# Julia-Tempering/Pigeons.jl

Hardware: AMD Instinct MI355X
Metric: replica-steps/sec (explore+swap), toy_mvn d=1024, n_chains=1024; round-trip rate (higher is better)
Workload: dtype f64

## Files before the change

include/pte.h:

```cpp
#ifndef PTE_H
#define PTE_H

#include <stdint.h>
#include "pte_rng_policy.h"

#ifdef __cplusplus
extern "C" {
#endif

#define PTE_ABI_VERSION 2

enum {
    PTE_TARGET_MVN_SCALED_PRECISION = 0,
    PTE_TARGET_TEST_SWAPPER         = 1,
    PTE_TARGET_FUNNEL               = 2,
    PTE_TARGET_ISING                = 3,
    PTE_TARGET_GAUSSIAN_MIXTURE     = 4,
    PTE_TARGET_BAYESIAN_GLM         = 5,
    PTE_TARGET_MIXTURE_MODEL        = 6,
    PTE_TARGET_VARIABLE_SELECTION = 7,
    PTE_TARGET_CHANGE_POINT = 8,
    PTE_TARGET_HIERARCHICAL_NORMAL = 9,
    PTE_TARGET_LATENT_AR1 = 10,
    PTE_TARGET_DENSE_NORMAL = 11,
// ... 23 lines not shown
    PTE_EXPLORER_CHECKERBOARD_METROPOLIS = 7
};
enum {
    PTE_RECORD_ROUND_TRIP    = 1u << 0,
    PTE_RECORD_INDEX_PROCESS = 1u << 1,
    PTE_RECORD_ONLINE        = 1u << 2,
    PTE_RECORD_TRACES        = 1u << 3,
    PTE_RECORD_TRACES_EXTENDED = 1u << 5,
    PTE_RECORD_ENERGY_AC1    = 1u << 4,
    PTE_RECORD_REFERENCE_REDUCTION = 1u << 6
};

enum {
    PTE_KERNEL_DEFAULT          = 0,
    PTE_KERNEL_SLICE_SEQUENTIAL = 1,
    PTE_KERNEL_ISING_BITS       = 101,
    PTE_KERNEL_ISING_BYTES      = 102,
    PTE_KERNEL_TWO_LAUNCHES     = 0x1000,
    PTE_KERNEL_SCAN_LOOP_ONE_CHAIN = 0x2000,
    PTE_KERNEL_FLAG_BITS        = 0x3000,
    PTE_KERNEL_TEST_DEAD_CHAIN     = 0x4000,
    PTE_KERNEL_TEST_LATE_WORKGROUP = 0x8000,
    PTE_KERNEL_TEST_LANGEVIN_ONE_WAVE = 0x10000,
    PTE_KERNEL_TEST_BITS        = 0x1C000
};

typedef struct pte_config {
    uint32_t struct_size;
    uint32_t abi_version;
    int32_t  device;
    int32_t  target;
    int32_t  explorer;
    uint32_t record_flags;
    int64_t  n_chains;
    int64_t  dim;
    uint64_t seed;
    int64_t  max_scans_per_round;
    double   target_params[4];
    double   slice_w;
    int32_t  slice_p;
    int32_t  slice_n_passes;
    int32_t  slice_max_iter;
    int32_t  am_base_n_refresh;
    double   am_exponent_n_refresh;
    double   am_step_size;
    double   am_p0, am_p1;
    int32_t  am_preconditioner;
// ... 70 lines not shown
int64_t pte_shard_message_bytes(const pte_engine *h);
int pte_shard_set_buffers(pte_engine *h, void *send_lo, void *recv_lo, void *send_hi, void *recv_hi);
int pte_shard_scan_begin(pte_engine *h, int64_t scan, int32_t *active_out);
int pte_shard_scan_finish(pte_engine *h, int64_t scan);
int pte_shard_sync(pte_engine *h, int64_t *boundary_swaps_out);
#define PTE_COMM_ID_BYTES 128
int pte_comm_allow_library_override(int32_t allow);
int pte_comm_library(char *path_out, int64_t capacity, int32_t *version_out);
int pte_comm_unique_id(uint8_t *id_out );
int pte_comm_init(pte_engine *h, const uint8_t *id );
int pte_comm_destroy(pte_engine *h);
int pte_comm_info(pte_engine *h, int32_t *kind, int32_t *n_ranks_seen, int64_t *boundary_swaps);
int pte_comm_barrier(pte_engine *h);
int pte_comm_allreduce(pte_engine *h, double *inout, int64_t n, int32_t op);
int pte_comm_allgather(pte_engine *h, const void *send, int64_t bytes, void *recv);
int pte_group_run_scans(pte_engine *const *engines, int32_t n_engines, int64_t first_scan, int64_t n_scans);

const char *pte_kernel_name(const pte_engine *h);

const char *pte_scan_loop_name(const pte_engine *h);
int pte_scan_loop_info(const pte_engine *h, int64_t *resident_limit, int64_t *timed_launches, int64_t *timed_scans);
int pte_scan_loop_stats(const pte_engine *h, int64_t *fused_calls, int64_t *gate_aborts, int32_t *poisoned);

int pte_get_index_process_shard(const pte_engine *h, int64_t *replica, int64_t *chain, int64_t *n_scans);
int pte_get_replica_ids(const pte_engine *h, int64_t *out );

int pte_timing_reset(pte_engine *h, int enable);
int pte_timing_get(const pte_engine *h, int kernel, double *total_ms, int64_t *launches);
int pte_timing_get_samples(const pte_engine *h, int kernel, double *out_ms, int64_t capacity, int64_t *n_out);

int pte_set_rng_policy(int32_t device, uint32_t policy);
int pte_get_rng_policy(int32_t device, uint32_t *policy);

int pte_test_rng_fill(int32_t device, uint64_t *seed_gamma , int32_t kind, int64_t n, double *out);
int pte_test_quotient(int32_t device, const double *a, const double *b, int64_t n, double *out, int32_t *took_division);
int pte_test_sqr_norm(int32_t device, const double *x, int64_t rows, int64_t d, double *out);

#ifdef __cplusplus
}
#endif
#endif
```

pigeons.jl_amd/csrc/pte.hip:

```cpp
#include <hip/hip_runtime.h>
#include <hip/hip_ext.h>

#include <cmath>
#include <cstdarg>
#include <cstdio>
#include <cstdlib>
#include <cstring>
#include <string>
#include <vector>

#include "../../include/pte.h"
#include "pte_kernels.hpp"
#include "pte_slice2.hpp"
#include "pte_slice5.hpp"
#include "pte_slice7.hpp"
#include "pte_slice8.hpp"
#ifdef PTE_SPLIT_LANGEVIN
#include "pte_automala_params.hpp"
#include "pte_aaps_params.hpp"
#include "pte_mixture_params.hpp"
#include "pte_glm_params.hpp"
#include "pte_hier_params.hpp"
#include "pte_ar1_params.hpp"
#include "pte_dense_params.hpp"
// ... 488 lines not shown
    hipLaunchKernelGGL(k_log_energy, dim3((unsigned)((N + 255) / 256)), dim3(256), 0, h->stream, h->dev, 1);
    HIP_OK(h, hipGetLastError());
    return 0;
}

int launch_explorer_kind(pte_engine *h, int64_t scan, int kind) {
    const int64_t N = h->K;
    switch (kind) {
    case PTE_EXPLORER_NONE: return 0;
    case PTE_EXPLORER_TOY:
        time_begin(h, 0, true);
        DISPATCH_NLU(h->nlu, k_explore_toy, dim3((unsigned)((N + NRM_WPB - 1) / NRM_WPB)), dim3(64 * NRM_WPB), h->stream, h->dev);
        time_end(h);
        break;
    case PTE_EXPLORER_SLICE:
        if (on_interpolated_path(h->cfg.target)) {
            const AmParams ap = slice_path_params(h);
            time_begin(h, 0, true);
            if (launch_path_kernel(h, blocks_per_lane(h->d), true, false, N, ap)) return 1;
            time_end(h);
            break;
        }
        {
        SliceParams sp{h->cfg.slice_w, h->cfg.slice_p, h->cfg.slice_n_passes, h->cfg.slice_max_iter};
        time_begin(h, 0, true);
        if (h->slice_impl == 1) {
            DISPATCH_NLU(h->nlu, k_explore_slice, dim3((unsigned)N), dim3(64), h->stream, h->dev, sp);
        } else if (h->slice_impl == 8) {
            const bool fast_ok = sp.p > PTE_S8_BD && sp.p <= 20 && sp.max_iter >= PTE_S8_BS;
            if (N <= PTE_S8_TWIN_FROM && fast_ok) { DISPATCH_NLU_M(h->nlu, k_explore_slice8, PTE_S8_BS, dim3((unsigned)N), dim3(64), h->stream, h->dev, sp); }
            else if (N <= PTE_S8_TWIN_FROM) { DISPATCH_NLU_M(h->nlu, k_explore_slice8_generic, PTE_S8_BS, dim3((unsigned)N), dim3(64), h->stream, h->dev, sp); }
            else { DISPATCH_NLU_M(h->nlu, k_explore_slice8_lds10k, PTE_S8_BS, dim3((unsigned)N), dim3(64), h->stream, h->dev, sp); }
        }
#ifdef PTE_TEST_KERNELS
        else if (h->slice_impl == 7) {
            S7Tune tn{2, 8, 2};
            DISPATCH_NLU(h->nlu, k_explore_slice7, dim3((unsigned)N), dim3(64), h->stream, h->dev, sp, tn);
        } else if (h->slice_impl == 5) {
            DISPATCH_NLU_M(h->nlu, k_explore_slice5, 4, dim3((unsigned)N), dim3(64), h->stream, h->dev, sp);
        } else if (h->slice_impl == 2) {
            DISPATCH_NLU_M(h->nlu, k_explore_slice2, 4, dim3((unsigned)N), dim3(64), h->stream, h->dev, sp);
        }
#endif
        else return fail(h, "SliceSampler kernel %d is not in this build", h->slice_impl);
        time_end(h);
        break;
    }
// ... 170 lines not shown
}

int run_scans_two_launches(pte_engine *h, int64_t first_scan, int64_t n_scans) {
    for (int64_t s = first_scan; s < first_scan + n_scans; ++s) {
        if (launch_explore(h, s)) return 1;
        if (launch_swap(h, s)) return 1;
    }
    int rc = check_device_error(h);
    time_collect(h);
    return rc;
}

int run_scans_fused(pte_engine *h, int64_t first_scan, int64_t n_scans) {
    const int64_t N = h->K;
    const int kind = fused_kind(h);
    const unsigned long long wgs = (unsigned long long)((kind == 2 && h->fused_wg > 1) ? (N + h->fused_wg - 1) / h->fused_wg : N);
    h->gate_seq += 1;
    ScanLoop sl{first_scan, n_scans, h->scans_in_round, h->hs_epoch, h->hs_flag, h->hs_pub, h->hs_gate, h->gate_seq, h->gate_arrived + wgs, h->test_fault};
    h->gate_arrived += wgs;
    h->dev.compose_phase = 0; h->dev.trace_idx = h->scans_in_round;
    time_begin(h, 4, true);
    const bool timed = h->ev_open;
    if (kind == 1) {
        SliceParams sp{h->cfg.slice_w, h->cfg.slice_p, h->cfg.slice_n_passes, h->cfg.slice_max_iter};
        if (fused_slice_variant(h) == 0) { DISPATCH_NLU_M(h->nlu, k_scans_slice8, PTE_S8_BS, dim3((unsigned)N), dim3(64), h->stream, h->dev, sp, sl); }
        else { DISPATCH_NLU_M(h->nlu, k_scans_slice8_generic, PTE_S8_BS, dim3((unsigned)N), dim3(64), h->stream, h->dev, sp, sl); }
    } else {
        const AmParams ap = langevin_params(h, h->cfg.explorer, 1);
        const int E = blocks_per_lane(h->d);
        LangevinLaunch L{E, h->cfg.target == PTE_TARGET_FUNNEL ? TGT_FUNNEL : TGT_MVN, false, h->d == 64 * (int64_t)E, launch_site(h, (unsigned)wgs)};
        L.scans = &sl; L.scan_wg = h->fused_wg;
        if (E == 16) HIP_OK(h, hipMemsetAsync(h->dev.pace, 0, sizeof(unsigned int), h->stream));
        if (langevin_launch(L, h->dev, ap)) { time_end(h); return fail(h, "this build holds no fused Langevin-family kernel"); }
    }
    time_end(h);
    HIP_OK(h, hipGetLastError());
    unsigned long long gate[2] = {0, 0};
    HIP_OK(h, hipMemcpyAsync(gate, h->hs_gate, sizeof gate, hipMemcpyDeviceToHost, h->stream));
    int rc = check_device_error(h);
    if (gate[1] == ((h->gate_seq << 1) | 1ull)) {
        if (timed && !h->events.empty() && h->events.back().kernel == 4) {
            h->ev_pool.push_back(h->events.back().a); h->ev_pool.push_back(h->events.back().b); h->events.pop_back();
        }
        h->gate_aborts += 1;
        h->fused_backoff = h->fused_backoff ? std::min<int64_t>(256, 2 * h->fused_backoff) : 1;
        h->fused_skip = h->fused_backoff;
        if (rc) return rc;
// ... 294 lines not shown
        auto composable = [&](int k) { return k == PTE_EXPLORER_SLICE || grad_based(k); };
        if (!composable(cfg->explorer) || !composable(cfg->explorer2))
            return fail(nullptr, "pte_create: Compose is available for SliceSampler / AutoMALA / MALA (got %d, %d)", cfg->explorer, cfg->explorer2);
    }
    if (!swapper && !ising && (cfg->dim < 1 || cfg->dim > 4096))
        return fail(nullptr, "pte_create: dim must be in 1..4096 (got %lld)", (long long)cfg->dim);
    if (swapper && cfg->explorer != PTE_EXPLORER_NONE)
        return fail(nullptr, "pte_create: TestSwapper has no explorer");
    if (!swapper && !ising && cfg->explorer != PTE_EXPLORER_TOY && cfg->explorer != PTE_EXPLORER_SLICE && !grad_based(cfg->explorer) && !aaps)
        return fail(nullptr, "pte_create: explorer %d is not implemented on the device", cfg->explorer);
    if ((cfg->record_flags & PTE_RECORD_TRACES_EXTENDED) && !(cfg->record_flags & PTE_RECORD_TRACES))
        return fail(nullptr, "pte_create: PTE_RECORD_TRACES_EXTENDED needs PTE_RECORD_TRACES");
    if (cfg->record_flags & PTE_RECORD_REFERENCE_REDUCTION) {
        if (!(cfg->record_flags & PTE_RECORD_INDEX_PROCESS))
            return fail(nullptr, "pte_create: PTE_RECORD_REFERENCE_REDUCTION needs PTE_RECORD_INDEX_PROCESS (the replay asks which replica held the lower chain of a pair)");
        if ((double)cfg->max_scans_per_round * (double)(cfg->n_chains + cfg->n_chains_variational) * 16.0 > 64e9)
            return fail(nullptr, "pte_create: the swap log (max_scans_per_round x chains x 2 doubles) would exceed 64 GB");
    }
#ifndef PTE_TEST_KERNELS
    if (cfg->debug_kernel & PTE_KERNEL_TEST_BITS)
        return fail(nullptr, "pte_create: debug_kernel 0x%x carries a fault-injection flag (PTE_KERNEL_TEST_*); those exist in the test build libpte_test.so only", cfg->debug_kernel);
#endif
    {
        const int dk = cfg->debug_kernel & ~(PTE_KERNEL_FLAG_BITS | PTE_KERNEL_TEST_BITS);
        const bool slice = cfg->explorer == PTE_EXPLORER_SLICE || cfg->explorer2 == PTE_EXPLORER_SLICE;
        bool ok = dk == 0 || (slice && dk == PTE_KERNEL_SLICE_SEQUENTIAL) || (ising && dk == PTE_KERNEL_ISING_BYTES);
#ifdef PTE_TEST_KERNELS
        ok = ok || (slice && (dk == 2 || dk == 5 || dk == 7 || dk == 8)) || (ising && !spin_glass && !checkerboard && dk == PTE_KERNEL_ISING_BITS);
#endif
        if (!ok) return fail(nullptr, "pte_create: debug_kernel %d is not available for this explorer in this build of libpte "
                                      "(0 = default, %d = sequential SliceSampler kernel; the other generations live in the test build libpte_test.so)",
                             dk, PTE_KERNEL_SLICE_SEQUENTIAL);
    }
    if ((cfg->record_flags & PTE_RECORD_TRACES) &&
        (double)cfg->max_scans_per_round * (double)((cfg->record_flags & PTE_RECORD_TRACES_EXTENDED) ? cfg->n_chains / cfg->world_size : 1) * (double)(cfg->dim + 1) * 8.0 > 64e9)
        return fail(nullptr, "pte_create: the traces buffer (max_scans_per_round x chains x (dim+1) doubles) would exceed 64 GB");
    return 0;
}

int poisoned_error(pte_engine *h, const char *what) {
    return fail(h, "%s: this engine is poisoned -- an earlier pte_run_scans failed inside the one-launch scan loop, its replicas stopped at different scans; "
                   "restore it with pte_set_state(state, chain, rng) or destroy it", what);
}
#define PTE_ALIVE(h, what) do { if ((h)->poisoned) return poisoned_error(h, what); } while (0)

int setter_entry(pte_engine *h, const char *setter, int32_t target, const char *wrong_target) {
    if (!h) return 1;
    PTE_ALIVE(h, setter);
// ... 53 lines not shown
const char *pte_last_error(const pte_engine *h) { return h ? h->err.c_str() : g_create_error.c_str(); }

int pte_create(const pte_config *cfg, pte_engine **out) {
    if (!cfg || !out) return fail(nullptr, "pte_create: null argument");
    *out = nullptr;
    if (validate_config(cfg)) return 1;
    int ndev = 0;
    if (hipGetDeviceCount(&ndev) != hipSuccess || ndev <= 0)
        return fail(nullptr, "pte_create: no HIP device available (this library has no CPU fallback)");
    if (cfg->device < 0 || cfg->device >= ndev) return fail(nullptr, "pte_create: bad device ordinal %d", cfg->device);

    pte_engine *h = new pte_engine();
    h->cfg = *cfg;
    const int64_t N = h->N = cfg->n_chains + cfg->n_chains_variational;
    const int64_t d = h->d = cfg->target == PTE_TARGET_TEST_SWAPPER ? 0 : cfg->dim;
    h->world = cfg->world_size; h->rank = cfg->rank;
    const int64_t K = h->K = N / cfg->world_size;
    h->c0 = K * cfg->rank;
    auto bail = [&](int) { g_create_error = h->err; pte_destroy(h); return 1; };
    if (hipSetDevice(cfg->device) != hipSuccess) { h->err = "hipSetDevice failed"; return bail(1); }
    if (hipStreamCreate(&h->stream) != hipSuccess) { h->err = "hipStreamCreate failed"; return bail(1); }
    const int64_t B = (d + 63) / 64;
    h->nlu = next_pow2_log(B > 0 ? B : 1);
    const int dk_kernel = cfg->debug_kernel & ~(PTE_KERNEL_FLAG_BITS | PTE_KERNEL_TEST_BITS);
    h->fused_allowed = (cfg->debug_kernel & PTE_KERNEL_TWO_LAUNCHES) == 0;
    h->fused_wg_allowed = (cfg->debug_kernel & PTE_KERNEL_SCAN_LOOP_ONE_CHAIN) == 0;
    h->test_fault = (cfg->debug_kernel & PTE_KERNEL_TEST_DEAD_CHAIN) ? 1 : ((cfg->debug_kernel & PTE_KERNEL_TEST_LATE_WORKGROUP) ? 2 : 0);
    if (cfg->explorer == PTE_EXPLORER_SLICE || cfg->explorer2 == PTE_EXPLORER_SLICE) h->slice_impl = dk_kernel == 0 ? 8 : dk_kernel;
    if (cfg->explorer == PTE_EXPLORER_ISING_METROPOLIS || cfg->explorer == PTE_EXPLORER_CHECKERBOARD_METROPOLIS) h->ising_impl = dk_kernel == PTE_KERNEL_ISING_BITS ? 1 : (dk_kernel == PTE_KERNEL_ISING_BYTES ? 2 : 0);
    if (alloc_engine(h)) return bail(1);
    default_schedule(h);
    if (upload_ladder(h)) return bail(1);
    if (reset_recorders(h)) return bail(1);
    if (init_replicas(h)) return bail(1);
    if ((on_interpolated_path(cfg->target) || on_lattice(cfg->target)) && init_zero_state(h)) return bail(1);
    *out = h;
    return 0;
}

int pte_destroy(pte_engine *h) {
    if (!h) return 0;
    hipSetDevice(h->cfg.device);
    if (h->stream) hipStreamSynchronize(h->stream);
    time_collect(h);
    pte_comm_destroy(h);
    if (h->ev_pack) hipEventDestroy(h->ev_pack);
    if (h->ev_copied) hipEventDestroy(h->ev_copied);
// ... 806 lines not shown
}

const char *pte_scan_loop_name(const pte_engine *hc) {
    pte_engine *h = const_cast<pte_engine *>(hc);
    if (!h) return "";
    hipSetDevice(h->cfg.device);
    if (!fused_scans_eligible(h, 1)) return "";
    if (fused_kind(h) == 2) return h->d > 512 ? "k_scans_langevin_mw" : h->fused_wg > 1 ? "k_scans_automala_wg" : "k_scans_automala";
    return fused_slice_variant(h) == 0 ? "k_scans_slice8" : "k_scans_slice8_generic";
}
int pte_scan_loop_info(const pte_engine *hc, int64_t *resident_limit, int64_t *timed_launches, int64_t *timed_scans) {
    pte_engine *h = const_cast<pte_engine *>(hc);
    if (!h) return 1;
    hipSetDevice(h->cfg.device);
    (void)fused_scans_eligible(h, 1);
    hipStreamSynchronize(h->stream);
    time_collect(h);
    if (resident_limit) *resident_limit = h->fused_limit < 0 ? 0 : h->fused_limit;
    if (timed_launches) *timed_launches = h->t_n[4];
    if (timed_scans) *timed_scans = h->t_scans4;
    return 0;
}

int pte_scan_loop_stats(const pte_engine *h, int64_t *fused_calls, int64_t *gate_aborts, int32_t *poisoned) {
    if (!h) return 1;
    if (fused_calls) *fused_calls = h->fused_calls;
    if (gate_aborts) *gate_aborts = h->gate_aborts;
    if (poisoned) *poisoned = h->poisoned ? 1 : 0;
    return 0;
}

int pte_set_target_mixture(pte_engine *h, int64_t n_components, const double *weights, const double *means, const double *std_devs) {
    if (setter_entry(h, "pte_set_target_mixture", PTE_TARGET_GAUSSIAN_MIXTURE, "pte_set_target_mixture: this engine's target is %d, not PTE_TARGET_GAUSSIAN_MIXTURE")) return 1;
    if (n_components < 1 || n_components > 8)
        return fail(h, "pte_set_target_mixture: the device holds 1..8 components (got %lld)", (long long)n_components);
    if (!weights || !means || !std_devs) return fail(h, "pte_set_target_mixture: null argument");
    const int64_t K = n_components, d = h->d, ld = h->dev.ld;
    for (int64_t k = 0; k < K; ++k) {
        if (!(weights[k] > 0) || !std::isfinite(weights[k]))
            return fail(h, "pte_set_target_mixture: weight %lld must be positive and finite (got %g)", (long long)k, weights[k]);
        for (int64_t i = 0; i < d; ++i) {
            const double sd = std_devs[k * d + i], mu = means[k * d + i];
            if (!(sd > 0) || !std::isfinite(sd))
                return fail(h, "pte_set_target_mixture: std_devs[%lld][%lld] must be positive and finite (got %g)", (long long)k, (long long)i, sd);
            if (!std::isfinite(mu))
                return fail(h, "pte_set_target_mixture: means[%lld][%lld] must be finite (got %g)", (long long)k, (long long)i, mu);
// ... 578 lines not shown
```

pigeons.jl_amd/csrc/pte_kernels.hpp:

```cpp
#pragma once
#include "pte_device.hpp"
#include "pte_normals.hpp"

namespace pte {

enum { ERR_NONE = 0, ERR_NAN_RATIO = 1, ERR_SLICE_SUPPORT = 2, ERR_SLICE_INVALID_LP = 3, ERR_SLICE_MAX_ITER = 4 };

struct EngineDev {
    int64_t N, d, ld;
    int64_t sw;
    int64_t K, c0;
    int64_t *replica_id;
    double *stat;
    double *nbr_stat;
    int32_t *bflag;
    int32_t *slot_of_chain_alt;
    int32_t *ip_replica;
    double *x;
    uint64_t *rng;
    int32_t *chain_of_slot;
    int32_t *slot_of_chain;
    double *suff;
    const double *nhp;
    const double *sd;
// ... 7 lines not shown
    double *swap_sum;  int64_t *swap_n;
    double *lsr_up;    double *lsr_dn;   int64_t *lsr_n;
    double *swap_log;
    int16_t *am_log; int am_log_cap;
    int64_t *rt_state; int64_t *rt_restarts; int64_t *rt_trips;
    double *expl_acc_sum; int64_t *expl_acc_n;
    double *expl_steps_sum; int64_t *expl_steps_n;
    double *on_mean; double *on_m2; int64_t *on_n;
    double *eac_log;
    double *eac; int64_t *eac_n;
    double *traces; int64_t trace_idx;
    int64_t ref2, tgt_a, tgt_b, rt_tgt_a, rt_tgt_b;
    const int32_t *v_use; const double *v_mean, *v_std, *v_c0, *v_i2, *v_gf; double *suff3;
    int compose_phase; double *lp_stash;
    int32_t *index_process;
    int32_t *error;
    double *mw_gk;
    unsigned int *pace;
    uint32_t record_flags;
    int32_t target;
    double test_swapper_pr;
};

struct SliceParams { double w; int p; int n_passes; int max_iter; };

__device__ __forceinline__ bool is_ref_chain(const EngineDev &e, int64_t c) { return (c == 0 && e.N > 1) || c == e.ref2; }
__device__ __forceinline__ bool is_tgt_chain(const EngineDev &e, int64_t c) { return c == e.tgt_a || c == e.tgt_b; }

__device__ __forceinline__ void set_error(const EngineDev &e, int code, int chain, int coord) {
    if (atomicCAS(&e.error[0], 0, code) == 0) { e.error[1] = chain; e.error[2] = coord; }
}

template <int NLU>
__global__ __launch_bounds__(64 * NRM_WPB) NRM_ATTR void k_init(EngineDev e, uint64_t master_seed, double init_sd) {
    __shared__ NormalsLds L;
    const int lane = lane_id();
    normals_lds_init(L, lane);
    const int64_t il = (int64_t)blockIdx.x * NRM_WPB + (NRM_WPB > 1 ? __builtin_amdgcn_readfirstlane((int)(threadIdx.x >> 6)) : 0);
    if (il >= e.K) return;
    const int64_t i = e.c0 + il;
    const uint64_t G = 0x9e3779b97f4a7c15ULL;
    SeqRng r;
    r.seed = mix64(master_seed + (uint64_t)(2 * i + 1) * G);
    r.gamma = mix_gamma(master_seed + (uint64_t)(2 * i + 2) * G);
    if (e.d > 0) {
        const double S = upper_tree_root<NLU>(normals_row(L, r, e.x + il * e.ld, e.d, init_sd, lane));
        if (lane == 0) e.suff[il] = S;
// ... 806 lines not shown
```

pigeons.jl_amd/csrc/pte_slice7.hpp:

```cpp
#pragma once
#include "pte_slice5.hpp"

namespace pte {

namespace s7 {
#ifndef PTE_S7_G
#define PTE_S7_G 5
#endif
constexpr int G = PTE_S7_G;
#ifndef PTE_S7_WIN
#define PTE_S7_WIN 512
#endif
constexpr int WIN = PTE_S7_WIN;
#ifndef PTE_S7_MARGIN
#define PTE_S7_MARGIN 80
#endif
constexpr int REFILL_AT = WIN - PTE_S7_MARGIN;
constexpr int CAP_ITERS = 24;
#ifndef PTE_S7_TABLES
#define PTE_S7_TABLES {0, 3, 6, 10, 14}, {1, 14, 16, 17, 16}, {0, 1, 15, 31, 48}
#endif
struct S7Tables { int lo[G], wd[G], base[G]; };
constexpr S7Tables S7T = {PTE_S7_TABLES};
struct S7Row { int v[G]; };
constexpr S7Row s7_row(const int (&a)[G]) { S7Row r{}; for (int i = 0; i < G; ++i) r.v[i] = a[i]; return r; }
__device__ constexpr S7Row LO_ = s7_row(S7T.lo), WD_ = s7_row(S7T.wd), BASE_ = s7_row(S7T.base);
#define LO LO_.v
#define WD WD_.v
#define BASE BASE_.v
__device__ __forceinline__ int s7_level(int lane) { int g = 0; for (int k = 1; k < G; ++k) g += (lane >= BASE[k]) ? 1 : 0; return g; }
__device__ __forceinline__ int s7_pick(const int (&a)[G], int g, int dflt) { int r = dflt; for (int k = 0; k < G; ++k) r = (g == k) ? a[k] : r; return r; }
constexpr int VALID = 1 << 30;
}

struct S7Tune { int bud_d, bud_s, bud_a; };
namespace s7 {
}

template <int NLU>
__global__ __launch_bounds__(64) void k_explore_slice7(EngineDev e, SliceParams sp, S7Tune tn) {
    using namespace s7;
    __shared__ double s_we[256];
    __shared__ unsigned long long s_ke[256];
    __shared__ double s_u[WIN];
    __shared__ double s_e[WIN];
    const int lane = lane_id();
    for (int i = lane; i < 256; i += 64) { s_we[i] = ZIG_WE[i]; s_ke[i] = ZIG_KE[i]; }
    __syncthreads();
    const int64_t cl = blockIdx.x;
    if (cl >= e.K) return;
    const int64_t c = e.c0 + cl;
    const int slot = e.slot_of_chain[cl];
// ... 294 lines not shown
```

pigeons.jl_amd/csrc/pte_slice8.hpp:

```cpp
#pragma once
#include "pte_slice7.hpp"

namespace pte {

#ifndef PTE_S8_BD
#define PTE_S8_BD 3
#endif
#ifndef PTE_S8_BS
#define PTE_S8_BS 9
#endif
constexpr int S8_BD = PTE_S8_BD;

#ifndef PTE_S8_WAVES
#define PTE_S8_WAVES 4
#endif
template <int NLU, int S8_BS, int WINDOW, int DBL_MODE>
__device__ __forceinline__ void slice8_body(EngineDev e, SliceParams sp, const int64_t cl) {
    using namespace s7;
    constexpr int WIN = WINDOW, REFILL_AT = WINDOW - PTE_S7_MARGIN;
    constexpr bool FAST = (DBL_MODE == 2);
    static_assert(CAP_ITERS >= S8_BS, "lane 0 must be able to run past the speculative budget");
#ifndef PTE_S8_BLK
#define PTE_S8_BLK 256
#endif
// ... 26 lines not shown
    __syncthreads();
    if (cl >= e.K) return;
    const int64_t c = e.c0 + cl;
    const int slot = e.slot_of_chain[cl];
    if (is_ref_chain(e, c)) {
        iid_refresh_recorded<NLU>(e, cl, c, slot, e.sd[c], lane);
        return;
    }
    const double lp_before = lp_before_explore(e, c, slot);
    const int64_t d = e.d;
    double *xrow = e.x + (int64_t)slot * e.ld;
    const int B = (int)((d + 63) >> 6);
    const double nhp = e.nhp[c];
    const double inv_nhp = 1.0 / nhp;
    const double inv_abs_nhp = -inv_nhp * (1.0 + 1e-6);
    const double w = sp.w;
    const double w11 = 1.1 * sp.w;
    const int cap_iters = min(sp.max_iter, CAP_ITERS);
    const int kcap = min(sp.p, 20);
    const bool shr_more = S8_BS < cap_iters;
    constexpr bool HAND_SHRINK = (S8_BS == PTE_S8_BS && S8_BS >= 6 && S8_BS <= 10);
    constexpr bool N_IS_KN = (DBL_MODE == 2) && HAND_SHRINK;

    const int hg = s7_level(lane);
    const int hrel = s7_pick(LO, hg, 0) + lane - s7_pick(BASE, hg, 0);

    const int succ_lo = s7_pick(LO, hg + 1, 0), succ_wd = s7_pick(WD, hg + 1, 0), succ_base = s7_pick(BASE, hg + 1, 0);
    const int succ_off = hrel - succ_lo;
    const int word_c = 0x10000 - succ_off;
    const int word_c9 = (1 << 20) - succ_off * 512;
    const uint64_t seed_in = e.rng[2 * slot];

    double BS = 0.0;
    for (int b = 0; b < B; ++b) {
        int64_t i = 64 * (int64_t)b + lane;
        double v = (i < d) ? xrow[i] : 0.0;
        double s = wave_sum_dpp(v * v);
        if (lane == b) BS = s;
    }
    double S = upper_tree_root<NLU>(BS);
    if (nhp * S == -INFINITY) { if (lane == 0) set_error(e, ERR_SLICE_SUPPORT, (int)c, -1); return; }

    uint64_t wseed = e.rng[2 * slot];
    const uint64_t gamma = e.rng[2 * slot + 1];
    int p = 0;
    uint64_t gamma_inv = gamma;
    for (int k = 0; k < 5; ++k) gamma_inv *= 2ull - gamma * gamma_inv;
    double wsum = 0.0;
    typedef unsigned mask2_t __attribute__((ext_vector_type(2)));
    typedef unsigned slow_mask_t __attribute__((ext_vector_type(WIN / 32)));
    typedef double draws8_t __attribute__((ext_vector_type(8)));
// ... 538 lines not shown
                                 : [sB] "=&s"(sB_), [tm] "=&s"(tmask), [acc] "=&s"(acc),
                                   [s0] "=&s"(s0_), [s1] "=&s"(s1_), [s2] "=&s"(s2_), [s3] "=&s"(s3_), [s4] "=&s"(s4_)
                                 : [w] "v"(w_), [pk] "v"(pk_)
                                 : "scc");
                    if (__builtin_amdgcn_inverse_ballot_w64(tmask)) s_x[(l + hg) & (BLK - 1)] = xf;
                    __builtin_amdgcn_wave_barrier();
                    p += (int)((acc >> 9) & 0x1FFu);
                    gdone = (int)((acc >> 20) & 7u);
                    l += gdone;
                } else {
                bool valid = __builtin_amdgcn_inverse_ballot_w64(pre_ok) && fin && (W > thr2);
                if constexpr (!FAST) valid = valid && !(E != E) && n <= cap_iters;
#ifdef PTE_PROFILE_SECTIONS
                asm volatile("" :: "v"(xf), "v"(n), "v"(dmin));
#endif
#ifdef PTE_PROFILE_SECTIONS
                {
                    const bool mg = dmin > 2e-12 * Bq;
                    const int rc = !active ? 7 : (E != E) ? 1 : !dbl_ok ? 2 : !fin ? 3 : !valid ? 4 : !mg ? 5 : 0;
                    const int cnt_ = N_IS_KN ? n - succ_off : cnt_base + kd + n;
                    int o_ = 0, g_ = 0, why = 0;
                    for (g_ = 0; g_ < G; ++g_) {
                        if (l + g_ >= nl) { why = 7; break; }
                        const int k_ = o_ - LO[g_];
                        if ((unsigned)k_ >= (unsigned)WD[g_]) { why = 6; break; }
                        const int ln_ = BASE[g_] + k_;
                        const int r_ = __builtin_amdgcn_readlane(rc, ln_);
                        if (r_) { why = r_; break; }
                        o_ += __builtin_amdgcn_readlane(cnt_, ln_);
                    }
                    PROF_ADD(8 + why, 1);
                }
#endif
                valid = valid && (dmin > mthr);
                const int kn = N_IS_KN ? n : kn0 + n;
                const bool inw = (unsigned)kn < (unsigned)succ_wd;
                const uint64_t vmask = ballot64(valid);
                int word_v = kn + word_c + (inw ? (int)((unsigned)(kn + succ_base) << 24) : 0);
                asm("" : "+v"(word_v));
                const int word = valid ? word_v : 0;
                const int packed = (lane != 0) ? word : 0;
#ifdef PTE_PROFILE_SECTIONS
                asm volatile("" :: "v"(packed));
#endif
                {
                    int pk = __builtin_amdgcn_readlane(word, 0);
                    unsigned acc = 0u;
                    uint64_t tmask = 1ull;
#pragma unroll
// ... 190 lines not shown
```

pigeons.jl_amd/pigeons_amd/_lib.py:

```python
import ctypes as C
import os

_HERE = os.path.dirname(os.path.abspath(__file__))
PKG_ROOT = os.path.dirname(_HERE)
LIB_PATH = os.path.join(PKG_ROOT, "lib", "libpte.so")


def use_library(path):
    global LIB_PATH
    LIB_PATH = path

TARGET_MVN_SCALED_PRECISION, TARGET_TEST_SWAPPER, TARGET_FUNNEL, TARGET_ISING, TARGET_GAUSSIAN_MIXTURE = 0, 1, 2, 3, 4
TARGET_BAYESIAN_GLM = 5
TARGET_MIXTURE_MODEL = 6
TARGET_VARIABLE_SELECTION = 7
TARGET_CHANGE_POINT = 8
TARGET_HIERARCHICAL_NORMAL = 9
HIER_CENTERED, HIER_NONCENTERED = 0, 1
TARGET_LATENT_AR1 = 10
AR1_STOCHASTIC_VOLATILITY, AR1_NORMAL_IDENTITY = 0, 1
TARGET_DENSE_NORMAL = 11
TARGET_SPIN_GLASS = 12
TARGET_SPIN_GLASS_3D = 13
CHANGEPOINT_FORM_AUTO, CHANGEPOINT_FORM_FULL, CHANGEPOINT_FORM_CACHED = 0, 1, 2
GLM_BERNOULLI_LOGIT, GLM_NORMAL_IDENTITY = 0, 1
EXPLORER_NONE, EXPLORER_TOY, EXPLORER_SLICE, EXPLORER_AUTOMALA, EXPLORER_ISING_METROPOLIS, EXPLORER_MALA, EXPLORER_AAPS = 0, 1, 2, 3, 4, 5, 6
EXPLORER_CHECKERBOARD_METROPOLIS = 7
RECORD_ROUND_TRIP, RECORD_INDEX_PROCESS, RECORD_ONLINE, RECORD_TRACES, RECORD_ENERGY_AC1, RECORD_TRACES_EXTENDED = 1, 2, 4, 8, 16, 32
RECORD_REFERENCE_REDUCTION = 64
ABI_VERSION = 2
KERNEL_DEFAULT, KERNEL_SLICE_SEQUENTIAL, KERNEL_ISING_BITS, KERNEL_ISING_BYTES = 0, 1, 101, 102
KERNEL_SCAN_LOOP_ONE_CHAIN = 0x2000
KERNEL_FLAG_BITS = 0x3000
KERNEL_TEST_DEAD_CHAIN, KERNEL_TEST_LATE_WORKGROUP, KERNEL_TEST_BITS = 0x4000, 0x8000, 0x1C000
KERNEL_TEST_LANGEVIN_ONE_WAVE = 0x10000
KERNEL_TWO_LAUNCHES = 0x1000
COMM_ID_BYTES = 128
RNG_TAIL_LOG1P = 1


def rng_bool_bit(k):
    return (k & 63) << 8
TEST_LIB_PATH = os.path.join(PKG_ROOT, "lib", "libpte_test.so")
NRMCUT_LIB_PATH = os.path.join(PKG_ROOT, "lib", "libpte_nrmcut.so")


class PteConfig(C.Structure):
    _fields_ = [
        ("struct_size", C.c_uint32), ("abi_version", C.c_uint32),
        ("device", C.c_int32), ("target", C.c_int32), ("explorer", C.c_int32),
        ("record_flags", C.c_uint32),
        ("n_chains", C.c_int64), ("dim", C.c_int64), ("seed", C.c_uint64),
        ("max_scans_per_round", C.c_int64),
        ("target_params", C.c_double * 4),
        ("slice_w", C.c_double),
        ("slice_p", C.c_int32), ("slice_n_passes", C.c_int32), ("slice_max_iter", C.c_int32),
        ("am_base_n_refresh", C.c_int32),
        ("am_exponent_n_refresh", C.c_double), ("am_step_size", C.c_double),
        ("am_p0", C.c_double), ("am_p1", C.c_double),
# ... 8 lines not shown


EXPORTS = [
    "pte_default_config", "pte_create", "pte_destroy", "pte_last_error",
    "pte_set_schedule", "pte_get_schedule", "pte_set_explorer_adaptation",
    "pte_explore", "pte_swap", "pte_run_scans", "pte_reduce",
    "pte_get_swap_acceptance", "pte_get_log_sum_ratio", "pte_get_round_trip",
    "pte_get_index_process", "pte_get_explorer_stats", "pte_get_automala_stats",
    "pte_get_online", "pte_get_state", "pte_set_state",
    "pte_timing_reset", "pte_timing_get", "pte_timing_get_samples", "pte_test_rng_fill", "pte_test_sqr_norm", "pte_test_quotient",
    "pte_shard_info", "pte_swap_begin", "pte_swap_finish", "pte_boundary_payload_bytes",
    "pte_boundary_export", "pte_boundary_import", "pte_get_index_process_shard", "pte_get_replica_ids",
    "pte_get_stream", "pte_shard_message_bytes", "pte_shard_set_buffers", "pte_shard_scan_begin",
    "pte_shard_scan_finish", "pte_shard_sync",
    "pte_get_online_log_density", "pte_get_energy_ac1", "pte_get_traces", "pte_set_variational_reference",
    "pte_comm_allow_library_override", "pte_comm_library", "pte_comm_unique_id", "pte_comm_init", "pte_comm_destroy", "pte_comm_info", "pte_comm_barrier",
    "pte_comm_allreduce", "pte_comm_allgather", "pte_group_run_scans", "pte_kernel_name",
    "pte_set_rng_policy", "pte_get_rng_policy", "pte_scan_loop_name", "pte_scan_loop_info", "pte_scan_loop_stats",
    "pte_set_target_mixture", "pte_set_target_glm", "pte_set_target_mixture_model", "pte_set_target_varsel",
    "pte_set_target_changepoint", "pte_set_changepoint_form", "pte_set_target_hier", "pte_set_target_ar1",
    "pte_set_target_dense",
    "pte_set_target_spin_glass",
    "pte_set_target_spin_glass_3d",
]

_libs = {}
_comm_override_allowed = False


def comm_allow_library_override(allow=True):
    global _comm_override_allowed
    _comm_override_allowed = bool(allow)
    for L in _libs.values():
        L.pte_comm_allow_library_override(1 if allow else 0)


def load(path=None):
    path = path or LIB_PATH
    if path in _libs:
        return _libs[path]
    if not os.path.exists(path):
        raise PteError(
            "HIP extension %s is missing: run `python -c 'import __graft_entry__ as g; g.build()'` "
            "(hipcc --offload-arch=gfx950). There is no CPU fallback." % path)
    try:
        import torch
# ... 61 lines not shown
    L.pte_shard_set_buffers.argtypes = [vp, C.c_void_p, C.c_void_p, C.c_void_p, C.c_void_p]
    L.pte_shard_scan_begin.argtypes = [vp, C.c_int64, i32p]
    L.pte_shard_scan_finish.argtypes = [vp, C.c_int64]
    L.pte_shard_sync.argtypes = [vp, ip]
    u8p = C.POINTER(C.c_uint8)
    L.pte_comm_allow_library_override.argtypes = [C.c_int32]
    L.pte_comm_library.argtypes = [C.c_char_p, C.c_int64, i32p]
    L.pte_comm_unique_id.argtypes = [u8p]
    L.pte_comm_init.argtypes = [vp, u8p]
    L.pte_comm_destroy.argtypes = [vp]
    L.pte_comm_info.argtypes = [vp, i32p, i32p, ip]
    L.pte_comm_barrier.argtypes = [vp]
    L.pte_comm_allreduce.argtypes = [vp, dp, C.c_int64, C.c_int32]
    L.pte_comm_allgather.argtypes = [vp, C.c_void_p, C.c_int64, C.c_void_p]
    L.pte_group_run_scans.argtypes = [C.POINTER(vp), C.c_int32, C.c_int64, C.c_int64]
    L.pte_set_rng_policy.argtypes = [C.c_int32, C.c_uint32]
    L.pte_get_rng_policy.argtypes = [C.c_int32, C.POINTER(C.c_uint32)]
    L.pte_kernel_name.argtypes = [vp]
    L.pte_kernel_name.restype = C.c_char_p
    L.pte_scan_loop_name.argtypes = [vp]
    L.pte_scan_loop_name.restype = C.c_char_p
    L.pte_scan_loop_info.argtypes = [vp, ip, ip, ip]
    L.pte_scan_loop_stats.argtypes = [vp, ip, ip, i32p]
    for name in EXPORTS:
        if name not in ("pte_last_error", "pte_boundary_payload_bytes", "pte_get_stream", "pte_shard_message_bytes", "pte_kernel_name", "pte_scan_loop_name"):
            getattr(L, name).restype = C.c_int
    if _comm_override_allowed:
        L.pte_comm_allow_library_override(1)
    _libs[path] = L
    return L
```

pigeons.jl_amd/pigeons_amd/pt.py:

```python
import time
from dataclasses import dataclass, field
from typing import Any, List, Optional

import numpy as np

from . import _lib
from .engine import Engine
from . import tempering as T


from .explorers import (AAPS, MALA, AutoMALA, CheckerboardMetropolis, Compose, DiagonalPreconditioner, IdentityPreconditioner,
                        IsingMetropolis, MixDiagonalPreconditioner, SliceSampler, ToyExplorer, engine_kw)
from .targets import (BayesianGLM, DenseNormal, Funnel, GaussianMixture, GaussianReference, HierarchicalNormalMeans, InterpolatingPath,
                      IsingLogPotential, LatentAR1, MixtureModelPosterior, PoissonChangePoint, ScaledPrecisionNormalLogPotential,
                      ScaledPrecisionNormalPath, SpikeSlabRegression, SpinGlass3DLogPotential, SpinGlassLogPotential, TestSwapper,
                      analytic_cumulativebarrier, analytic_lognormalization, default_explorer, toy_mvn_target)


def log_sum_ratio(): return "log_sum_ratio"
def swap_acceptance_pr(): return "swap_acceptance_pr"
def round_trip(): return "round_trip"
def index_process(): return "index_process"
def online(): return "online"
def traces(): return "traces"
# ... 122 lines not shown
        self.reduced_recorders = ReducedRecorders()
        names = {b() for b in inputs.record}
        flags = 0
        for name, flag in RECORD_FLAGS.items():
            if name in names:
                flags |= flag
        if "traces" in names and getattr(inputs, "extended_traces", False):
            flags |= _lib.RECORD_TRACES_EXTENDED
        if reference_reduction:
            flags |= _lib.RECORD_REFERENCE_REDUCTION | _lib.RECORD_INDEX_PROCESS
        if inputs.variational is not None:
            if not isinstance(inputs.variational, GaussianReference) or not getattr(target, "takes_gaussian_reference", False):
                raise NotImplementedError("the device engine has GaussianReference on the interpolated (funnel) path only")
            flags |= _lib.RECORD_ONLINE
        kw = dict(device=inputs.device, n_chains=N, n_chains_variational=n_var, seed=inputs.seed, record_flags=flags,
                  max_scans_per_round=2 ** inputs.n_rounds)
        if not hasattr(target, "device_family"):
            raise NotImplementedError("target %r has no device log-potential; use the reference CPU path (Pigeons.jl)" % (target,))
        kw.update(target.device_family(inputs, explorer))
        kw.update(engine_kw(explorer))
        make = engine_factory or Engine
        if debug_kernel:
            kw.update(debug_kernel=debug_kernel)
            if (debug_kernel & ~(_lib.KERNEL_FLAG_BITS | _lib.KERNEL_TEST_BITS)) not in (0, _lib.KERNEL_SLICE_SEQUENTIAL, _lib.KERNEL_ISING_BYTES) or (debug_kernel & _lib.KERNEL_TEST_BITS):
                kw.update(test_build=True)
        self.shards = None
        if n_shards > 1:
            from .sharded import LoopbackShards
            self.shards = LoopbackShards([make(rank=g, world_size=n_shards, **kw) for g in range(n_shards)], device_messages=device_messages,
                                         transport=transport)
            self.replicas = self.shards.engines[0]
        elif world > 1:
            from .sharded import DistShard, RcclShard
            self.replicas = make(rank=rank, world_size=world, **kw)
            if transport != "host" and hasattr(self.replicas, "comm_init"):
                self.shards = RcclShard(self.replicas, rank, world, id_bytes=comm_id)
            else:
                self.shards = DistShard(self.replicas, rank, world, device=dist_device)
        else:
            self.replicas = make(**kw)
        if hasattr(target, "upload"):
            for eng in (self.shards.engines if hasattr(self.shards, "engines") else [self.replicas]):
                target.upload(eng)

def next_round(pt):
    it = pt.shared.iterators
    if it.round + 1 <= pt.inputs.n_rounds:
# ... 254 lines not shown
```

Before: 1.749 million.

## Select slice8 window layout per chain from slice width and precision

Adds multiple lane-to-level window layouts for the slice8 kernel when G==5 and WINDOW==512. Each chain picks one at runtime from rho2 = w^2 * (-2*nhp), or a debug_kernel bit field forces the choice. The lane tables for all layouts are computed and packed into one register. The idea is that the stepping-out and shrink search resolves in one round more often for chains whose scale differs. The cost is extra per-lane setup arithmetic, table indexing in the resolve loop, and more host-side validation plus a new query API.

```diff
diff --git a/include/pte.h b/include/pte.h
--- a/include/pte.h
+++ b/include/pte.h
@@ -69,7 +69,9 @@
     PTE_KERNEL_TEST_DEAD_CHAIN     = 0x4000,
     PTE_KERNEL_TEST_LATE_WORKGROUP = 0x8000,
     PTE_KERNEL_TEST_LANGEVIN_ONE_WAVE = 0x10000,
-    PTE_KERNEL_TEST_BITS        = 0x1C000
+    PTE_KERNEL_TEST_BITS        = 0x1C000,
+    PTE_KERNEL_SLICE8_LAYOUT_SHIFT = 17,
+    PTE_KERNEL_SLICE8_LAYOUT_MASK  = 0x60000
 };
 
 typedef struct pte_config {
@@ -186,6 +188,8 @@
 int pte_scan_loop_info(const pte_engine *h, int64_t *resident_limit, int64_t *timed_launches, int64_t *timed_scans);
 int pte_scan_loop_stats(const pte_engine *h, int64_t *fused_calls, int64_t *gate_aborts, int32_t *poisoned);
 
+int pte_slice8_layout(int32_t k, double w, double nhp, int32_t *rows, int32_t *n_layouts, int32_t *chain_class);
+
 int pte_get_index_process_shard(const pte_engine *h, int64_t *replica, int64_t *chain, int64_t *n_scans);
 int pte_get_replica_ids(const pte_engine *h, int64_t *out );
 
diff --git a/pigeons.jl_amd/csrc/pte.hip b/pigeons.jl_amd/csrc/pte.hip
--- a/pigeons.jl_amd/csrc/pte.hip
+++ b/pigeons.jl_amd/csrc/pte.hip
@@ -534,7 +534,7 @@
             break;
         }
         {
-        SliceParams sp{h->cfg.slice_w, h->cfg.slice_p, h->cfg.slice_n_passes, h->cfg.slice_max_iter};
+        SliceParams sp{h->cfg.slice_w, h->cfg.slice_p, h->cfg.slice_n_passes, h->cfg.slice_max_iter, (h->cfg.debug_kernel & PTE_KERNEL_SLICE8_LAYOUT_MASK) >> PTE_KERNEL_SLICE8_LAYOUT_SHIFT};
         time_begin(h, 0, true);
         if (h->slice_impl == 1) {
             DISPATCH_NLU(h->nlu, k_explore_slice, dim3((unsigned)N), dim3(64), h->stream, h->dev, sp);
@@ -751,7 +751,7 @@
     time_begin(h, 4, true);
     const bool timed = h->ev_open;
     if (kind == 1) {
-        SliceParams sp{h->cfg.slice_w, h->cfg.slice_p, h->cfg.slice_n_passes, h->cfg.slice_max_iter};
+        SliceParams sp{h->cfg.slice_w, h->cfg.slice_p, h->cfg.slice_n_passes, h->cfg.slice_max_iter, (h->cfg.debug_kernel & PTE_KERNEL_SLICE8_LAYOUT_MASK) >> PTE_KERNEL_SLICE8_LAYOUT_SHIFT};
         if (fused_slice_variant(h) == 0) { DISPATCH_NLU_M(h->nlu, k_scans_slice8, PTE_S8_BS, dim3((unsigned)N), dim3(64), h->stream, h->dev, sp, sl); }
         else { DISPATCH_NLU_M(h->nlu, k_scans_slice8_generic, PTE_S8_BS, dim3((unsigned)N), dim3(64), h->stream, h->dev, sp, sl); }
     } else {
@@ -1092,8 +1092,13 @@
         return fail(nullptr, "pte_create: debug_kernel 0x%x carries a fault-injection flag (PTE_KERNEL_TEST_*); those exist in the test build libpte_test.so only", cfg->debug_kernel);
 #endif
     {
-        const int dk = cfg->debug_kernel & ~(PTE_KERNEL_FLAG_BITS | PTE_KERNEL_TEST_BITS);
+        const int dk = cfg->debug_kernel & ~(PTE_KERNEL_FLAG_BITS | PTE_KERNEL_TEST_BITS | PTE_KERNEL_SLICE8_LAYOUT_MASK);
         const bool slice = cfg->explorer == PTE_EXPLORER_SLICE || cfg->explorer2 == PTE_EXPLORER_SLICE;
+        const int forced_layout = (cfg->debug_kernel & PTE_KERNEL_SLICE8_LAYOUT_MASK) >> PTE_KERNEL_SLICE8_LAYOUT_SHIFT;
+        if (forced_layout > s7::N_LAYOUTS)
+            return fail(nullptr, "pte_create: debug_kernel 0x%x forces window layout %d of the slice8 kernels, which hold %d (pte_slice8_layout)", cfg->debug_kernel, forced_layout - 1, s7::N_LAYOUTS);
+        if (forced_layout != 0 && !(slice && !family && (dk == 0 || dk == 8)))
+            return fail(nullptr, "pte_create: debug_kernel 0x%x forces a window layout, which only SliceSampler's default kernel on the scaled-precision MVN path has", cfg->debug_kernel);
         bool ok = dk == 0 || (slice && dk == PTE_KERNEL_SLICE_SEQUENTIAL) || (ising && dk == PTE_KERNEL_ISING_BYTES);
 #ifdef PTE_TEST_KERNELS
         ok = ok || (slice && (dk == 2 || dk == 5 || dk == 7 || dk == 8)) || (ising && !spin_glass && !checkerboard && dk == PTE_KERNEL_ISING_BITS);
@@ -1193,7 +1198,7 @@
     if (hipStreamCreate(&h->stream) != hipSuccess) { h->err = "hipStreamCreate failed"; return bail(1); }
     const int64_t B = (d + 63) / 64;
     h->nlu = next_pow2_log(B > 0 ? B : 1);
-    const int dk_kernel = cfg->debug_kernel & ~(PTE_KERNEL_FLAG_BITS | PTE_KERNEL_TEST_BITS);
+    const int dk_kernel = cfg->debug_kernel & ~(PTE_KERNEL_FLAG_BITS | PTE_KERNEL_TEST_BITS | PTE_KERNEL_SLICE8_LAYOUT_MASK);
     h->fused_allowed = (cfg->debug_kernel & PTE_KERNEL_TWO_LAUNCHES) == 0;
     h->fused_wg_allowed = (cfg->debug_kernel & PTE_KERNEL_SCAN_LOOP_ONE_CHAIN) == 0;
     h->test_fault = (cfg->debug_kernel & PTE_KERNEL_TEST_DEAD_CHAIN) ? 1 : ((cfg->debug_kernel & PTE_KERNEL_TEST_LATE_WORKGROUP) ? 2 : 0);
@@ -2046,6 +2051,15 @@
     return 0;
 }
 
+int pte_slice8_layout(int32_t k, double w, double nhp, int32_t *rows, int32_t *n_layouts, int32_t *chain_class) {
+    if (n_layouts) *n_layouts = s7::N_LAYOUTS;
+    if (chain_class) *chain_class = s7::s7_layout_class(w, nhp);
+    if (!rows) return 0;
+    if (k < 0 || k >= s7::N_LAYOUTS) return 1;
+    for (int g = 0; g < s7::G; ++g) { rows[g] = s7::S7_LAYOUTS[k].lo[g]; rows[s7::G + g] = s7::S7_LAYOUTS[k].wd[g]; rows[2 * s7::G + g] = s7::S7_LAYOUTS[k].base[g]; }
+    return 0;
+}
+
 int pte_scan_loop_stats(const pte_engine *h, int64_t *fused_calls, int64_t *gate_aborts, int32_t *poisoned) {
     if (!h) return 1;
     if (fused_calls) *fused_calls = h->fused_calls;
diff --git a/pigeons.jl_amd/csrc/pte_kernels.hpp b/pigeons.jl_amd/csrc/pte_kernels.hpp
--- a/pigeons.jl_amd/csrc/pte_kernels.hpp
+++ b/pigeons.jl_amd/csrc/pte_kernels.hpp
@@ -53,7 +53,7 @@
     double test_swapper_pr;
 };
 
-struct SliceParams { double w; int p; int n_passes; int max_iter; };
+struct SliceParams { double w; int p; int n_passes; int max_iter; int layout; };
 
 __device__ __forceinline__ bool is_ref_chain(const EngineDev &e, int64_t c) { return (c == 0 && e.N > 1) || c == e.ref2; }
 __device__ __forceinline__ bool is_tgt_chain(const EngineDev &e, int64_t c) { return c == e.tgt_a || c == e.tgt_b; }
diff --git a/pigeons.jl_amd/csrc/pte_slice7.hpp b/pigeons.jl_amd/csrc/pte_slice7.hpp
--- a/pigeons.jl_amd/csrc/pte_slice7.hpp
+++ b/pigeons.jl_amd/csrc/pte_slice7.hpp
@@ -28,6 +28,39 @@
 #define LO LO_.v
 #define WD WD_.v
 #define BASE BASE_.v
+#if PTE_S7_G == 5
+#define PTE_S7_LAYOUT_LIST {{PTE_S7_TABLES}, {{0, 3, 6, 12, 18}, {1, 15, 17, 16, 15}, {0, 1, 16, 33, 49}}, {{0, 3, 7, 13, 19}, {1, 15, 17, 16, 15}, {0, 1, 16, 33, 49}}}
+#define PTE_S7_RHO2_BOUND_LIST {324.0, 784.0}
+constexpr int N_LAYOUTS = 3;
+#else
+#define PTE_S7_LAYOUT_LIST {{PTE_S7_TABLES}}
+#define PTE_S7_RHO2_BOUND_LIST {0.0}
+constexpr int N_LAYOUTS = 1;
+#endif
+constexpr S7Tables S7_LAYOUTS[N_LAYOUTS] = PTE_S7_LAYOUT_LIST;
+__device__ constexpr S7Tables S7_LAYOUTS_DEV[N_LAYOUTS] = PTE_S7_LAYOUT_LIST;
+constexpr double S7_RHO2_BOUNDS[N_LAYOUTS > 1 ? N_LAYOUTS - 1 : 1] = PTE_S7_RHO2_BOUND_LIST;
+constexpr bool s7_layout_ok(const S7Tables &t) {
+    int sum = 0;
+    bool ok = t.lo[0] == 0 && t.wd[0] == 1;
+    for (int g = 0; g < G; ++g) {
+        ok = ok && t.base[g] == sum && t.wd[g] >= 1 && t.lo[g] + t.wd[g] - 1 + 2 + 20 + CAP_ITERS <= PTE_S7_MARGIN;
+        sum += t.wd[g];
+    }
+    return ok && sum == 64;
+}
+constexpr bool s7_layouts_ok() {
+    for (int k = 0; k < N_LAYOUTS; ++k) if (!s7_layout_ok(S7_LAYOUTS[k])) return false;
+    for (int k = 1; k + 1 < N_LAYOUTS; ++k) if (!(S7_RHO2_BOUNDS[k - 1] < S7_RHO2_BOUNDS[k])) return false;
+    return true;
+}
+static_assert(s7_layouts_ok(), "a window layout breaks the round's assumptions (lane 0 certain, levels tile 64 lanes, reads inside PTE_S7_MARGIN)");
+__host__ __device__ inline int s7_layout_class(double w, double nhp) {
+    const double rho2 = w * w * (-2.0 * nhp);
+    int k = 0;
+    for (int j = 0; j + 1 < N_LAYOUTS; ++j) k += (rho2 >= S7_RHO2_BOUNDS[j]) ? 1 : 0;
+    return k;
+}
 __device__ __forceinline__ int s7_level(int lane) { int g = 0; for (int k = 1; k < G; ++k) g += (lane >= BASE[k]) ? 1 : 0; return g; }
 __device__ __forceinline__ int s7_pick(const int (&a)[G], int g, int dflt) { int r = dflt; for (int k = 0; k < G; ++k) r = (g == k) ? a[k] : r; return r; }
 constexpr int VALID = 1 << 30;
diff --git a/pigeons.jl_amd/csrc/pte_slice8.hpp b/pigeons.jl_amd/csrc/pte_slice8.hpp
--- a/pigeons.jl_amd/csrc/pte_slice8.hpp
+++ b/pigeons.jl_amd/csrc/pte_slice8.hpp
@@ -72,11 +72,31 @@
     constexpr bool HAND_SHRINK = (S8_BS == PTE_S8_BS && S8_BS >= 6 && S8_BS <= 10);
     constexpr bool N_IS_KN = (DBL_MODE == 2) && HAND_SHRINK;
 
-    const int hg = s7_level(lane);
-    const int hrel = s7_pick(LO, hg, 0) + lane - s7_pick(BASE, hg, 0);
-
-    const int succ_lo = s7_pick(LO, hg + 1, 0), succ_wd = s7_pick(WD, hg + 1, 0), succ_base = s7_pick(BASE, hg + 1, 0);
-    const int succ_off = hrel - succ_lo;
+    constexpr int NLAY = (WINDOW == 512) ? N_LAYOUTS : 1;
+    int lay = 0;
+    if constexpr (NLAY > 1) lay = (sp.layout > 0) ? sp.layout - 1 : s7_layout_class(sp.w, nhp);
+
+    int hg, hrel, succ_wd, succ_base, succ_off;
+    if constexpr (NLAY == 1) {
+        hg = s7_level(lane);
+        hrel = s7_pick(LO, hg, 0) + lane - s7_pick(BASE, hg, 0);
+        succ_wd = s7_pick(WD, hg + 1, 0); succ_base = s7_pick(BASE, hg + 1, 0);
+        succ_off = hrel - s7_pick(LO, hg + 1, 0);
+    } else {
+        int lpk = 0;
+#pragma unroll
+        for (int k = 0; k < NLAY; ++k) {
+            const S7Tables &T = S7_LAYOUTS_DEV[k];
+            int g = 0;
+            for (int j = 1; j < G; ++j) g += (lane >= T.base[j]) ? 1 : 0;
+            const int rel = s7_pick(T.lo, g, 0) + lane - s7_pick(T.base, g, 0);
+            const int pk = g | (rel << 3) | (s7_pick(T.wd, g + 1, 0) << 10) | (s7_pick(T.base, g + 1, 0) << 16) | ((rel - s7_pick(T.lo, g + 1, 0) + 64) << 24);
+            lpk = ((k == 0) || (lay == k)) ? pk : lpk;
+        }
+        asm volatile("" : "+v"(lpk));
+        hg = lpk & 7; hrel = (lpk >> 3) & 127; succ_wd = (lpk >> 10) & 63; succ_base = (lpk >> 16) & 255;
+        succ_off = ((lpk >> 24) & 255) - 64;
+    }
     const int word_c = 0x10000 - succ_off;
     const int word_c9 = (1 << 20) - succ_off * 512;
     const uint64_t seed_in = e.rng[2 * slot];
@@ -661,9 +681,10 @@
                     int o_ = 0, g_ = 0, why = 0;
                     for (g_ = 0; g_ < G; ++g_) {
                         if (l + g_ >= nl) { why = 7; break; }
-                        const int k_ = o_ - LO[g_];
-                        if ((unsigned)k_ >= (unsigned)WD[g_]) { why = 6; break; }
-                        const int ln_ = BASE[g_] + k_;
+                        const S7Tables &T_ = S7_LAYOUTS_DEV[lay < NLAY ? lay : 0];
+                        const int k_ = o_ - T_.lo[g_];
+                        if ((unsigned)k_ >= (unsigned)T_.wd[g_]) { why = 6; break; }
+                        const int ln_ = T_.base[g_] + k_;
                         const int r_ = __builtin_amdgcn_readlane(rc, ln_);
                         if (r_) { why = r_; break; }
                         o_ += __builtin_amdgcn_readlane(cnt_, ln_);
diff --git a/pigeons.jl_amd/pigeons_amd/_lib.py b/pigeons.jl_amd/pigeons_amd/_lib.py
--- a/pigeons.jl_amd/pigeons_amd/_lib.py
+++ b/pigeons.jl_amd/pigeons_amd/_lib.py
@@ -35,6 +35,7 @@
 KERNEL_TEST_DEAD_CHAIN, KERNEL_TEST_LATE_WORKGROUP, KERNEL_TEST_BITS = 0x4000, 0x8000, 0x1C000
 KERNEL_TEST_LANGEVIN_ONE_WAVE = 0x10000
 KERNEL_TWO_LAUNCHES = 0x1000
+KERNEL_SLICE8_LAYOUT_SHIFT, KERNEL_SLICE8_LAYOUT_MASK = 17, 0x60000
 COMM_ID_BYTES = 128
 RNG_TAIL_LOG1P = 1
 
@@ -89,6 +90,7 @@
     "pte_set_target_dense",
     "pte_set_target_spin_glass",
     "pte_set_target_spin_glass_3d",
+    "pte_slice8_layout",
 ]
 
 _libs = {}
@@ -196,6 +198,7 @@
     L.pte_scan_loop_name.restype = C.c_char_p
     L.pte_scan_loop_info.argtypes = [vp, ip, ip, ip]
     L.pte_scan_loop_stats.argtypes = [vp, ip, ip, i32p]
+    L.pte_slice8_layout.argtypes = [C.c_int32, C.c_double, C.c_double, i32p, i32p, i32p]
     for name in EXPORTS:
         if name not in ("pte_last_error", "pte_boundary_payload_bytes", "pte_get_stream", "pte_shard_message_bytes", "pte_kernel_name", "pte_scan_loop_name"):
             getattr(L, name).restype = C.c_int
diff --git a/pigeons.jl_amd/pigeons_amd/pt.py b/pigeons.jl_amd/pigeons_amd/pt.py
--- a/pigeons.jl_amd/pigeons_amd/pt.py
+++ b/pigeons.jl_amd/pigeons_amd/pt.py
@@ -168,7 +168,7 @@
         make = engine_factory or Engine
         if debug_kernel:
             kw.update(debug_kernel=debug_kernel)
-            if (debug_kernel & ~(_lib.KERNEL_FLAG_BITS | _lib.KERNEL_TEST_BITS)) not in (0, _lib.KERNEL_SLICE_SEQUENTIAL, _lib.KERNEL_ISING_BYTES) or (debug_kernel & _lib.KERNEL_TEST_BITS):
+            if (debug_kernel & ~(_lib.KERNEL_FLAG_BITS | _lib.KERNEL_TEST_BITS | _lib.KERNEL_SLICE8_LAYOUT_MASK)) not in (0, _lib.KERNEL_SLICE_SEQUENTIAL, _lib.KERNEL_ISING_BYTES) or (debug_kernel & _lib.KERNEL_TEST_BITS):
                 kw.update(test_build=True)
         self.shards = None
         if n_shards > 1:
```

New measurement: 1.721 million. 0.984x the previous value.
